# aj-prime/Elemental

Measured on AMD Instinct MI355X. Metric: distributed Gemm TFLOP/s (fp64/fp32) at 1/2/4/8 GPUs; % of MFMA peak, higher is better.
Workload: dtype f64; 1 GPU; C2: El::Gemm NN f64 m=n=k=32768, Grid 1x1; m=32768, n=32768, k=32768, grid=1x1, algorithm=SUMMA_C, blocksize=128, compute_panel=auto, parallelism=grid1x1, comm_reserved_cus=0

## Files before the change

### elemental_amd/_lib.py

```python
from __future__ import annotations

import ctypes
import os
from ctypes import (CFUNCTYPE, POINTER, c_char_p, c_double, c_float, c_int, c_int64, c_size_t,
                    c_ubyte, c_uint16, c_uint64, c_void_p)

_HERE = os.path.dirname(os.path.abspath(__file__))
LIB_PATH = os.path.join(_HERE, "libelemental_amd.so")

OK, ERR_LOGIC, ERR_HIP, ERR_COMM, ERR_RUNTIME, ERR_UNSUPPORTED, ERR_NO_DEVICE, ERR_SINGULAR = range(8)
ERR_NOT_HPD = 8
NORMAL, TRANSPOSE, ADJOINT = 0, 1, 2
MC, MD, MR, VC, VR, STAR, CIRC = range(7)
(GEMM_DEFAULT, GEMM_SUMMA_A_MS, GEMM_SUMMA_A, GEMM_SUMMA_B_MS, GEMM_SUMMA_B, GEMM_SUMMA_C_MS,
 GEMM_SUMMA_C, GEMM_SUMMA_DOT, GEMM_CANNON) = range(9)
ROW_MAJOR, COLUMN_MAJOR = 0, 1
LOWER, UPPER = 0, 1
LEFT, RIGHT = 0, 1
NON_UNIT, UNIT = 0, 1
CPU, GPU = 0, 1
F32, F64, F16, BF16 = 0, 1, 2, 3
I32, I64, U8 = 4, 5, 6
OP_SUM, OP_PROD, OP_MAX, OP_MIN = 0, 1, 2, 3
(MAP_IDENTITY, MAP_NEGATE, MAP_ABS, MAP_SQUARE, MAP_SQRT, MAP_EXP, MAP_LOG, MAP_RELU, MAP_SIGMOID,
 MAP_RECIP, MAP_TANH) = range(11)
(COMBINE_ADD, COMBINE_SUB, COMBINE_MUL, COMBINE_DIV, COMBINE_MAX, COMBINE_MIN, COMBINE_RELU_GRAD) = range(7)
FILE_AUTO, FILE_BINARY, FILE_BINARY_FLAT = 0, 3, 4
COLL_ALLGATHER, COLL_REDUCE_SCATTER, COLL_ALLTOALL, COLL_SENDRECV, COLL_BCAST, COLL_ALLREDUCE, \
    COLL_BARRIER = range(7)

HOST_COLL_FN = CFUNCTYPE(c_int, c_void_p, c_int, c_int, c_int, c_void_p, c_void_p, c_int64, c_int, c_int)
HOST_SPLIT_FN = CFUNCTYPE(c_int, c_void_p, c_int, c_int, c_int, POINTER(c_int), POINTER(c_int), POINTER(c_int))

_vp, _i, _i64, _d = c_void_p, c_int, c_int64, c_double
_SIGS = {
    "elx_last_error": (c_char_p, []),
    "elx_last_nonhpd_column": (_i, []),
    "elx_version": (_i, []),
    "elx_device_count": (_i, [POINTER(c_int)]),
    "elx_set_device": (_i, [_i]),
    "elx_get_device": (_i, [POINTER(c_int)]),
    "elx_device_synchronize": (_i, []),
    "elx_default_stream": (_i, [POINTER(c_void_p)]),
    "elx_comm_stream": (_i, [POINTER(c_void_p)]),
    "elx_reserved_cus": (_i, [POINTER(c_int)]),
    "elx_stream_create": (_i, [POINTER(c_void_p)]),
    "elx_stream_destroy": (_i, [_vp]),
    "elx_stream_synchronize": (_i, [_vp]),
    "elx_default_event": (_i, [POINTER(c_void_p)]),
    "elx_event_create": (_i, [POINTER(c_void_p)]),
    "elx_event_destroy": (_i, [_vp]),
    "elx_event_record": (_i, [_vp, _vp]),
    "elx_stream_wait_event": (_i, [_vp, _vp]),
    "elx_event_synchronize": (_i, [_vp]),
    "elx_pool_alloc": (_i, [POINTER(c_void_p), c_size_t, _vp]),
    "elx_pool_free": (_i, [_vp, _vp]),
    "elx_pool_trim": (_i, [c_size_t]),
    "elx_pool_stats": (_i, [POINTER(c_size_t), POINTER(c_size_t)]),
    "elx_pool_set_max_cached": (_i, [c_size_t]),
    "elx_pool_max_cached": (_i, [POINTER(c_size_t)]),
    "elx_pool_bin_bytes": (c_size_t, [c_size_t]),
    "elx_pool_bin_cacheable": (_i, [c_size_t]),
    "elx_pool_backing_reserved": (_i, [POINTER(c_size_t)]),
    "elx_memcpy_h2d": (_i, [_vp, _vp, c_size_t, _vp]),
    "elx_memcpy_d2h": (_i, [_vp, _vp, c_size_t, _vp]),
    "elx_memcpy_d2d": (_i, [_vp, _vp, c_size_t, _vp]),
    "elx_gemm_f64": (_i, [_i, _i, _i64, _i64, _i64, _d, _vp, _i64, _vp, _i64, _d, _vp, _i64, _vp]),
    "elx_gemm_f32": (_i, [_i, _i, _i64, _i64, _i64, c_float, _vp, _i64, _vp, _i64, c_float, _vp, _i64, _vp]),
# ... 218 lines not shown
```

### elemental_amd/csrc/capi.cpp

```cpp
#include "common.hpp"
#include "runtime/runtime.hpp"
#include "comm/comm.hpp"
#include "core/distmatrix.hpp"
#include "core/redist.hpp"
#include "core/gemm.hpp"
#include "core/lu.hpp"
#include "core/qr.hpp"
#include "core/random.hpp"
#include "core/io.hpp"
#include "core/exec.hpp"
#include <functional>
#include <string>

struct elx_comm_s { std::shared_ptr<elx::Comm> c; };
struct elx_grid_s { std::shared_ptr<elx::Grid> g; };
struct elx_dm_s { std::shared_ptr<elx::DistMatrix> m; };
struct elx_perm_s { elx::Permutation p; };

namespace elx {
namespace {
thread_local std::string g_last_error;

Dist ToDist(int d) {
    if (d < ELX_MC || d > ELX_CIRC) throw LogicError(Cat("invalid dist ", d));
// ... 29 lines not shown
using namespace elx;

extern "C" {

const char* elx_last_error(void) { return g_last_error.c_str(); }
int elx_last_nonhpd_column(void) { return g_last_nonhpd_column; }
int elx_version(void) { return 10000; }

int elx_device_count(int* count) {
    return Guard([&] {
        int n = 0;
        if (hipGetDeviceCount(&n) != hipSuccess) n = 0;
        *count = n;
    });
}
int elx_set_device(int device) { return Guard([&] { Runtime::Get().SetDevice(device); Runtime::Get().EnsureGPU(); }); }
int elx_get_device(int* device) { return Guard([&] { Runtime::Get().EnsureGPU(); *device = Runtime::Get().DeviceId(); }); }
int elx_device_synchronize(void) {
    return Guard([&] { Runtime::Get().EnsureGPU(); ELX_CHECK_HIP(hipDeviceSynchronize()); });
}
int elx_default_stream(void** stream) { return Guard([&] { *stream = Runtime::Get().ComputeStream(); }); }
int elx_comm_stream(void** stream) { return Guard([&] { *stream = Runtime::Get().CommStream(); }); }
int elx_reserved_cus(int* cus) { return Guard([&] { *cus = Runtime::Get().ReservedCUs(); }); }
int elx_stream_create(void** stream) {
    return Guard([&] {
        Runtime::Get().EnsureGPU();
        hipStream_t s;
        ELX_CHECK_HIP(hipStreamCreateWithFlags(&s, hipStreamNonBlocking));
        *stream = s;
    });
}
int elx_stream_destroy(void* stream) { return Guard([&] { ELX_CHECK_HIP(hipStreamDestroy(static_cast<hipStream_t>(stream))); }); }
int elx_stream_synchronize(void* stream) { return Guard([&] { ELX_CHECK_HIP(hipStreamSynchronize(S(stream))); }); }
int elx_default_event(void** event) {
    return Guard([&] {
        Runtime::Get().EnsureGPU();
        static hipEvent_t ev = [] {
            hipEvent_t e;
            ELX_CHECK_HIP(hipEventCreateWithFlags(&e, hipEventDisableTiming));
            return e;
        }();
        *event = ev;
    });
}
int elx_event_create(void** event) {
    return Guard([&] {
// ... 900 lines not shown
```

### elemental_amd/csrc/core/gemm.cpp

```cpp
#include "level3_internal.hpp"
#include <cstdlib>
#include "exec.hpp"
#include <algorithm>
#include <functional>
#include "../runtime/trace.hpp"
#include <vector>

namespace elx {

using namespace detail;

namespace {
std::vector<Int>& BlocksizeStack() {
    static std::vector<Int> s{128};
    return s;
}
Int g_compute_panel = 0;
int g_last_alg = ELX_GEMM_DEFAULT;
constexpr Int kDotBlock = 2000;
constexpr Int kDotBlockGPU = 2048;
Int DotBlockGPU() {
    static const Int v = [] { const char* e = getenv("ELX_DOT_BLOCK"); return e ? (Int)atoll(e) : kDotBlockGPU; }();
    return v;
}
// ... 125 lines not shown
        }
    }
};

int TeamCount(const DistMatrix& C, Int panels) {
    const int pool = StreamPoolSize();
    if (C.Dev() != Device::GPU || pool <= 1) return 1;
    return static_cast<int>(std::max<Int>(1, std::min<Int>(pool, panels)));
}

Int EffectivePanel(const Grid& g, Int K, DType t) {
    const Int nb = std::max<Int>(1, Blocksize());
    Int kc = g_compute_panel;
    const bool h16 = t == DType::F16 || t == DType::BF16;
    if (kc <= 0)
        kc = (g.Size() == 1) ? K : std::min<Int>(8192, std::max<Int>(2048, h16 ? K / 4 : K / 8));
    kc = std::max<Int>(nb, (kc + nb - 1) / nb * nb);
    return std::max<Int>(1, kc);
}

}

namespace detail {
void FenceStreams(hipStream_t from, hipStream_t to) {
    if (!from || !to || from == to) return;
    hipEvent_t ev;
    ELX_CHECK_HIP(hipEventCreateWithFlags(&ev, hipEventDisableTiming));
    ELX_CHECK_HIP(hipEventRecord(ev, from));
    ELX_CHECK_HIP(hipStreamWaitEvent(to, ev, 0));
    ELX_CHECK_HIP(hipEventDestroy(ev));
}

std::shared_ptr<const DistMatrix> ReadProxy(const DistMatrix& A, const DistMatrix& tgt, Dist cd, Dist rd,
                                            int calign, int ralign) {
    const bool ok = A.Dev() == tgt.Dev() && A.ColDist() == cd && A.RowDist() == rd &&
                    (calign < 0 || A.ColAlign() == calign) && (ralign < 0 || A.RowAlign() == ralign);
    if (ok) {
        if (A.Dev() != Device::GPU || A.Stream() == tgt.Stream())
            return std::shared_ptr<const DistMatrix>(&A, [](const DistMatrix*) {});
        auto V = DistMatrix::View(A, 0, A.Height(), 0, A.Width());
        V->SetStream(tgt.Stream());
        return V;
    }
    auto T = A.LikeOn(cd, rd, tgt.Dev());
    T->SetStream(tgt.Stream());
    const int ca = calign >= 0 ? calign : 0, ra = ralign >= 0 ? ralign : 0;
// ... 193 lines not shown
        const Int m = C.LocalHeight(), n = C.LocalWidth();
        const Int k = IsN(oA) ? a.LocalWidth() : a.LocalHeight();
        const double b_p = p == 0 ? beta : 1.0;
        if (m > 0 && n > 0 && k > 0) {
            const bool prof = gpu && Prof().on;
            Profiler::Rec rec{};
            if (prof) rec = Prof().Begin(cs);
            if (uplo >= 0)
                TrrkLocal(uplo == ELX_LOWER, !IsN(oA), !IsN(oB), k, alpha, a.Buffer(), a.LDim(), b.Buffer(), b.LDim(),
                          C, cs, trrk_tmp);
            else
                exec::Gemm(dev, C.Type(), !IsN(oA), !IsN(oB), m, n, k, alpha, a.Buffer(), a.LDim(), b.Buffer(),
                           b.LDim(), b_p, C.Buffer(), C.LDim(), cs);
            if (prof) Prof().End(rec, cs, 2.0 * m * n * k, Prof().gemm, call_id);
        } else if (p == 0) {
            Scale(beta, C);
        }
        if (gpu) {
            ELX_CHECK_HIP(hipEventRecord(s.done, cs));
            s.pending = true;
        }
    };
    if (np == 0) Scale(beta, C);
    if (np > 0) issue(0);
    for (int p = 0; p < np; ++p) {
        if (p + 1 < np) issue(p + 1);
        compute(p);
    }
    if (gpu) {
        FenceStreams(cs, ms);
        for (auto& s : slot) {
            s.ua.reset();
            s.ub.reset();
            s.va.reset();
            s.vb.reset();
            s.a.reset();
            s.b.reset();
            ELX_CHECK_HIP(hipEventDestroy(s.ready));
            ELX_CHECK_HIP(hipEventDestroy(s.done));
        }
    }
    Cp.Finish();
}
}

namespace {
// ... 12 lines not shown
    TeamViews tv(*Ap, *Bp, C0, TeamCount(C0, np));
    const int S = static_cast<int>(tv.v.size());
    const Dist a_cd = IsN(oA) ? Dist::MC : Dist::STAR, a_rd = IsN(oA) ? Dist::STAR : Dist::MC;
    const Dist b_cd = IsN(oB) ? Dist::STAR : Dist::MR, b_rd = IsN(oB) ? Dist::MR : Dist::STAR;
    struct TeamData { std::shared_ptr<DistMatrix> c, a, b; };
    std::vector<TeamData> td(S);
    for (int t = 0; t < S; ++t) {
        const DistMatrix& Ct = *tv.v[t].C;
        if (t == 0) {
            td[t].c = tv.v[t].C;
        } else {
            td[t].c = Ct.Like(Dist::MC, Dist::MR);
            td[t].c->Align(Ct.ColAlign(), Ct.RowAlign(), true);
            td[t].c->Resize(Ct.Height(), Ct.Width());
            Zero(*td[t].c);
        }
        td[t].a = tv.v[t].A->Like(a_cd, a_rd);
        td[t].b = tv.v[t].B->Like(b_cd, b_rd);
        if (IsN(oA)) td[t].a->AlignCols(Ct.ColAlign(), true); else td[t].a->AlignRows(Ct.ColAlign(), true);
        if (IsN(oB)) td[t].b->AlignRows(Ct.RowAlign(), true); else td[t].b->AlignCols(Ct.RowAlign(), true);
    }
    const Device dev = C0.Dev();
    const int call_id = Prof().calls++;
    for (Int p = 0; p < np; ++p) {
        const int t = static_cast<int>(p % S);
        const auto& v = tv.v[t];
        const DistMatrix& A = *v.A;
        const DistMatrix& B = *v.B;
        DistMatrix& Ct = *td[t].c;
        const Int k0 = p * kc, k1 = std::min(K, k0 + kc);
        auto Av = IsN(oA) ? DistMatrix::View(A, 0, A.Height(), k0, k1) : DistMatrix::View(A, k0, k1, 0, A.Width());
        auto Bv = IsN(oB) ? DistMatrix::View(B, k0, k1, 0, B.Width()) : DistMatrix::View(B, 0, B.Height(), k0, k1);
        std::shared_ptr<const DistMatrix> ua = Av, ub = Bv;
        if (!SameLocalLayout(*Av, a_cd, a_rd, td[t].a->ColAlign(), td[t].a->RowAlign())) {
            Copy(*Av, *td[t].a);
            ua = td[t].a;
        }
        if (!SameLocalLayout(*Bv, b_cd, b_rd, td[t].b->ColAlign(), td[t].b->RowAlign())) {
            Copy(*Bv, *td[t].b);
            ub = td[t].b;
        }
        const Int m = Ct.LocalHeight(), n = Ct.LocalWidth();
        const Int k = IsN(oA) ? ua->LocalWidth() : ua->LocalHeight();
        if (m > 0 && n > 0 && k > 0) {
            const bool prof = dev == Device::GPU && Prof().on;
            Profiler::Rec rec{};
// ... 355 lines not shown
```

### elemental_amd/csrc/kernels/gemm_f64g.hip

```cpp
#include <hip/hip_runtime.h>
#include <cstdint>
#include <cstdlib>
#include <type_traits>
#include "kernels.hpp"
#include "lds_dma.hpp"

namespace elx {
namespace kern {

namespace {

typedef double f64x4 __attribute__((ext_vector_type(4)));

constexpr int BK = 16, GROUP_M = 8;
constexpr bool RING64_DEFAULT = true;
template <int BM_, int WTM_ = 32, int SK_ = BK, int BN_ = 128, int WTN_ = 64>
struct Shape {
    static constexpr int BM = BM_, WTM = WTM_, MI = WTM_ / 16, WM = BM_ / WTM_, SK = SK_;
    static constexpr int BN = BN_, WTN = WTN_, NI = WTN_ / 16, WN = BN_ / WTN_, NW = WM * WN, NT = 64 * NW;
    static constexpr int IMGA = BM * SK * 8, IMGB = BN * SK * 8, STAGE = IMGA + IMGB;
    static constexpr int WAVES_PER_EU = BM_ == 64 && BN_ == 64 ? 4 : NW * (BM_ <= 128 && SK_ == 16 ? 2 : 1) / 4;
};

template <int SK>
__device__ __forceinline__ int swz_kc(int r) { return SK == 16 ? (r >> 1) & 7 : r & 15; }

struct GParams {
    i64 m, n, k;
    double alpha, beta;
    const double* A; i64 lda;
    const double* B; i64 ldb;
    double* C; i64 ldc;
    int tiles_m, tiles_n;
    i64 kchunk, zstride;
    int group_m;
    int xcd_remap;
};

__device__ __forceinline__ void tile_of(int bid, int nwg, int tiles_m, int tiles_n, int group_m, int remap, int& tm,
                                        int& tn) {
    const int xcd = bid & 7, q = nwg >> 3, r = nwg & 7;
    const int wg = remap ? (xcd < r ? xcd * (q + 1) : r * (q + 1) + (xcd - r) * q) + (bid >> 3) : bid;
    const int per_group = group_m * tiles_n;
    const int group = wg / per_group;
    const int first_m = group * group_m;
    const int gsz = min(tiles_m - first_m, group_m);
    const int inner = wg - group * per_group;
    tm = first_m + inner % gsz;
    tn = inner / gsz;
}

template <bool BUF, bool KC, int ROWS, int NW, int SK>
__device__ __forceinline__ void stage_img(const double* X, i64 ld, i64 rows, i64 R, i64 k0, lds_char* img, int w,
                                          int l) {
    constexpr int NINS = ROWS * SK * 8 / 1024;
    constexpr int CPR = SK / 2, RPI = 64 / CPR;
    const DmaSrc<BUF, double> src(KC ? X + R * ld + k0 : X + R + k0 * ld, (KC ? ROWS : SK) * ld * 8);
#pragma unroll
    for (int q = 0; q < NINS / NW; ++q) {
// ... 221 lines not shown
        if constexpr (NP > 0) {
            if (i >= H + OFF && (i - H - OFF) % SP == 0 && (i - H - OFF) / SP < NP) {
                const int u = u0 + (i - H - OFF) / SP;
                if constexpr (SB) piece<BT, UN, BUF, KCB>(p.B, p.ldb, n0, k0, pc.offB[u], pc.gB[u], w + 4 * u, st);
                else piece<BT, UN, BUF, KCA>(p.A, p.lda, m0, k0, pc.offA[u], pc.gA[u], w + 4 * u, st);
            }
        }
        __builtin_amdgcn_sched_barrier(0);
    }
}
}

template <int BT, int UN, bool KCA, bool KCB, bool BETA0, bool BUF>
__global__ __launch_bounds__(256, (ring::RG<BT, UN>::MINB)) void gemm_f64r_kernel(GParams p) {
    using namespace ring;
    using G = RG<BT, UN>;
    constexpr int RBK = G::RBK, UNIT = G::UNIT, WT = G::WT, MI = G::MI, NKS = G::NKS, NPW = G::NPW;
    constexpr int NPA = NPW / (NKS / 2);
    __shared__ __attribute__((aligned(1024))) char lds_raw[NSLOT * UNIT];
    lds_char* lds = (lds_char*)lds_raw;
    const int tid = threadIdx.x, l = tid & 63;
    const int w = __builtin_amdgcn_readfirstlane(tid >> 6);
    const int wr = w >> 1, wc = w & 1;
    int tm, tn;
    tile_of(blockIdx.x, gridDim.x, p.tiles_m, p.tiles_n, p.group_m, p.xcd_remap, tm, tn);
    const i64 m0 = (i64)tm * BT, n0 = (i64)tn * BT;
    {
        const i64 kz0 = (i64)blockIdx.y * p.kchunk;
        p.k = min(p.kchunk, p.k - kz0);
        p.A += KCA ? kz0 : kz0 * p.lda;
        p.B += KCB ? kz0 : kz0 * p.ldb;
        p.C += (i64)blockIdx.y * p.zstride;
    }
    Pieces<BT, UN> pc;
#pragma unroll
    for (int u = 0; u < NPW; ++u) {
        pc.gA[u] = piece_off<BT, UN, KCA>(w + 4 * u, l, m0, p.m, p.lda);
        pc.gB[u] = piece_off<BT, UN, KCB>(w + 4 * u, l, n0, p.n, p.ldb);
        pc.offA[u] = (int)(pc.gA[u] * 8);
        pc.offB[u] = (int)(pc.gB[u] * 8);
    }
    f64x4 acc[MI][MI];
#pragma unroll
    for (int a = 0; a < MI; ++a)
#pragma unroll
        for (int b = 0; b < MI; ++b) acc[a][b] = f64x4{0, 0, 0, 0};

    const int nt = (int)(p.k / RBK);
    auto kt = [&](int t) { return (i64)min(t, nt - 1) * RBK; };
#pragma unroll
    for (int t = 0; t < 2; ++t) {
#pragma unroll
        for (int u = 0; u < NPW; ++u)
            piece<BT, UN, BUF, KCA>(p.A, p.lda, m0, kt(t), pc.offA[u], pc.gA[u], w + 4 * u, lds + 2 * t * UNIT);
#pragma unroll
        for (int u = 0; u < NPW; ++u)
            piece<BT, UN, BUF, KCB>(p.B, p.ldb, n0, kt(t), pc.offB[u], pc.gB[u], w + 4 * u, lds + (2 * t + 1) * UNIT);
    }
    wait_cnt<2 * NPW, NOWAIT_LGKM>();
    dma_barrier();
    Ops<BT, UN> X, Y;
#pragma unroll
    for (int q = 0; q < MI; ++q) {
        X.a[q] = ropnd<BT, UN, KCA>(lds, wr * WT + q * 16, 0, l);
        X.b[q] = ropnd<BT, UN, KCB>(lds + UNIT, wc * WT + q * 16, 0, l);
    }
    wait_cnt<NOWAIT_VM, 0>();
    auto ktile = [&](auto jc, int t) {
        constexpr int J = decltype(jc)::value;
        constexpr int sA = 2 * J % NSLOT, sB = (2 * J + 1) % NSLOT, sA1 = (2 * J + 2) % NSLOT,
                      sB1 = (2 * J + 3) % NSLOT, st0 = (2 * J + 4) % NSLOT, st1 = (2 * J + 5) % NSLOT;
        lds_char* rA = lds + sA * UNIT;
        lds_char* rB = lds + sB * UNIT;
        const i64 k2 = kt(t + 2);
        auto ks = [&](auto sc) {
            constexpr int S = decltype(sc)::value;
            constexpr int NP = S < NKS / 2 ? NPA : 0;
            if constexpr (S % 2 == 0)
                ring::kstep<BT, UN, KCA, KCB, BUF, false, NP>(p, m0, n0, w, l, wr, wc, pc, rA, rB, S + 1,
                                                          lds + st0 * UNIT, S * NPA, k2, acc, X, Y);
            else
                ring::kstep<BT, UN, KCA, KCB, BUF, false, NP>(p, m0, n0, w, l, wr, wc, pc, rA, rB, S + 1,
                                                          lds + st0 * UNIT, S * NPA, k2, acc, Y, X);
            if constexpr (S < NKS - 2) wait_cnt<NOWAIT_VM, 0>();
        };
        ks(std::integral_constant<int, 0>{});
        ks(std::integral_constant<int, 1>{});
        ks(std::integral_constant<int, 2>{});
        if constexpr (NKS == 8) {
            ks(std::integral_constant<int, 3>{});
            ks(std::integral_constant<int, 4>{});
            ks(std::integral_constant<int, 5>{});
            ks(std::integral_constant<int, 6>{});
        }
        wait_cnt<NPW, 0>();
        dma_barrier();
        ring::kstep<BT, UN, KCA, KCB, BUF, true, NPW>(p, m0, n0, w, l, wr, wc, pc, lds + sA1 * UNIT, lds + sB1 * UNIT,
                                                  0, lds + st1 * UNIT, 0, k2, acc, Y, X);
        wait_cnt<NOWAIT_VM, 0>();
    };
    for (int t = 0; t < nt; t += NSLOT) {
        ktile(std::integral_constant<int, 0>{}, t);
        if (t + 1 < nt) ktile(std::integral_constant<int, 1>{}, t + 1);
        if (t + 2 < nt) ktile(std::integral_constant<int, 2>{}, t + 2);
        if (t + 3 < nt) ktile(std::integral_constant<int, 3>{}, t + 3);
        if (t + 4 < nt) ktile(std::integral_constant<int, 4>{}, t + 4);
    }
    asm volatile("s_waitcnt vmcnt(0)" ::: "memory");

    const int g = l >> 4, c = l & 15;
    const i64 ib = m0 + wr * WT + c, jb = n0 + wc * WT + g;
    if (m0 + BT <= p.m && n0 + BT <= p.n) {
#pragma unroll
        for (int mi = 0; mi < MI; ++mi) {
            double cv[MI][4];
            if (!BETA0) {
#pragma unroll
                for (int ni = 0; ni < MI; ++ni)
#pragma unroll
                    for (int r = 0; r < 4; ++r) cv[ni][r] = p.C[(jb + ni * 16 + 4 * r) * p.ldc + ib + mi * 16];
            }
#pragma unroll
            for (int ni = 0; ni < MI; ++ni)
#pragma unroll
                for (int r = 0; r < 4; ++r) {
                    const double v = p.alpha * acc[mi][ni][r];
                    p.C[(jb + ni * 16 + 4 * r) * p.ldc + ib + mi * 16] = BETA0 ? v : v + p.beta * cv[ni][r];
                }
        }
        return;
    }
#pragma unroll
    for (int mi = 0; mi < MI; ++mi)
#pragma unroll
        for (int ni = 0; ni < MI; ++ni) {
            const i64 i = ib + mi * 16;
            if (i >= p.m) continue;
#pragma unroll
            for (int r = 0; r < 4; ++r) {
                const i64 j = jb + ni * 16 + 4 * r;
                if (j < p.n) {
                    const double v = p.alpha * acc[mi][ni][r];
                    double* cp = p.C + j * p.ldc + i;
                    *cp = BETA0 ? v : v + p.beta * *cp;
                }
            }
        }
}

template <typename K>
hipError_t launch(K kernel, dim3 grid, int nt, const GParams& p, hipStream_t s) {
    hipLaunchKernelGGL(kernel, grid, dim3(nt), 0, s, p);
    return hipGetLastError();
}


template <typename SH, bool KCA, bool KCB, bool BUF>
hipError_t launch_b(const GParams& p, dim3 grid, hipStream_t s) {
    if (p.beta == 0.0) return launch(gemm_f64g_kernel<SH, KCA, KCB, true, BUF>, grid, SH::NT, p, s);
    return launch(gemm_f64g_kernel<SH, KCA, KCB, false, BUF>, grid, SH::NT, p, s);
}

template <typename SH, bool KCA, bool KCB>
hipError_t launch_g(GParams p, hipStream_t s) {
    p.tiles_m = (int)((p.m + SH::BM - 1) / SH::BM);
    p.tiles_n = (int)((p.n + SH::BN - 1) / SH::BN);
    const dim3 grid(p.tiles_m * p.tiles_n, (unsigned)((p.k + p.kchunk - 1) / p.kchunk));
    static const bool global_only = [] { const char* v = getenv("ELX_F64G_STAGE"); return v && v[0] == 'g'; }();
    if (!global_only && dma_fits(KCA ? SH::BM : SH::SK, p.lda, 8) && dma_fits(KCB ? SH::BN : SH::SK, p.ldb, 8))
        return launch_b<SH, KCA, KCB, true>(p, grid, s);
    return launch_b<SH, KCA, KCB, false>(p, grid, s);
}

template <int BT, int UN, bool KCA, bool KCB>
hipError_t launch_r(GParams p, hipStream_t s) {
    constexpr int RBK = ring::RG<BT, UN>::RBK;
    p.tiles_m = (int)((p.m + BT - 1) / BT);
    p.tiles_n = (int)((p.n + BT - 1) / BT);
    const dim3 grid(p.tiles_m * p.tiles_n, (unsigned)((p.k + p.kchunk - 1) / p.kchunk));
    const char* stg = getenv("ELX_F64G_STAGE");
    const bool buf = !(stg && stg[0] == 'g') && dma_fits(KCA ? BT : RBK, p.lda, 8) &&
                     dma_fits(KCB ? BT : RBK, p.ldb, 8);
    if (p.beta == 0.0) {
        if (buf) return launch(gemm_f64r_kernel<BT, UN, KCA, KCB, true, true>, grid, 256, p, s);
        return launch(gemm_f64r_kernel<BT, UN, KCA, KCB, true, false>, grid, 256, p, s);
    }
    if (buf) return launch(gemm_f64r_kernel<BT, UN, KCA, KCB, false, true>, grid, 256, p, s);
    return launch(gemm_f64r_kernel<BT, UN, KCA, KCB, false, false>, grid, 256, p, s);
}

template <typename SH>
hipError_t launch_shape(bool kca, bool kcb, const GParams& p, hipStream_t s) {
    if (kca) return kcb ? launch_g<SH, true, true>(p, s) : launch_g<SH, true, false>(p, s);
    return kcb ? launch_g<SH, false, true>(p, s) : launch_g<SH, false, false>(p, s);
}

bool al16(const void* q) { return (reinterpret_cast<uintptr_t>(q) & 15) == 0; }

bool t64_tiles(i64 m, i64 n, i64 k) {
    static const int v = [] { const char* e = getenv("ELX_F64G_T64"); return e ? atoi(e) : 1; }();
    if (v == 1 && (m + 127) / 128 * ((n + 127) / 128) == 256 && k / 32 * 32 <= 4096) return true;
    return prefer_t64(v, m, n, 255);
}

int ring_bt(i64 m, i64 n, i64 k) {
    const char* e = getenv("ELX_F64G_RING");
    const int v = e ? atoi(e) : RING64_DEFAULT ? 3 : 1;
    if (t64_tiles(m, n, k)) return (v & 2) ? 64 : 0;
    return (v & 1) ? 128 : 0;
}

}

DmaPlan gemm_f64_lds_dma_plan(bool ta, bool tb, i64 m, i64 n, i64 k, const double* A, i64 lda, const double* B,
                              i64 ldb) {
    const bool kca = ta, kcb = !tb;
    const bool ok = k >= BK && al16(A) && al16(B) && lda % 2 == 0 && ldb % 2 == 0 && (kca || (m % 2 == 0 && m >= 2)) &&
                    (kcb || (n % 2 == 0 && n >= 2)) && m < (1ll << 31) && n < (1ll << 31);
    const int bt = ring_bt(m, n, k);
    if (bt == 128) return dma_plan(ok && k >= 32, (m + 127) / 128 * ((n + 127) / 128), k, 32, 256);
    if (t64_tiles(m, n, k)) return dma_plan(ok, (m + 63) / 64 * ((n + 63) / 64), k, BK, bt == 64 ? 1024 : 512);
    return dma_plan(ok, (m + 127) / 128 * ((n + 127) / 128), k, BK);
}

hipError_t gemm_f64_lds_dma(bool ta, bool tb, i64 m, i64 n, i64 kmain, i64 kchunk, double alpha, const double* A,
                            i64 lda, const double* B, i64 ldb, double beta, double* C, i64 ldc, hipStream_t s) {
    static const int gm = [] {
        const char* v = getenv("ELX_F64G_GROUP");
        const int g = v ? atoi(v) : GROUP_M;
        return g >= 1 ? g : 1;
    }();
    static const int rm = [] { const char* v = getenv("ELX_F64G_REMAP"); return v ? atoi(v) : 1; }();
    GParams p{m, n, kmain, alpha, beta, A, lda, B, ldb, C, ldc, 0, 0, kchunk, m * n, gm, rm};
    static const int t64w = [] { const char* v = getenv("ELX_F64G_T64W"); return v ? atoi(v) : 0; }();
    const int bt = ring_bt(m, n, kmain);
    if (bt == 128 && kmain % 32 == 0 && kchunk % 32 == 0) {
        if (ta) return !tb ? launch_r<128, 32768, true, true>(p, s) : launch_r<128, 32768, true, false>(p, s);
        return !tb ? launch_r<128, 32768, false, true>(p, s) : launch_r<128, 32768, false, false>(p, s);
    }
    if (bt == 64 && kmain % 16 == 0 && kchunk % 16 == 0) {
        if (ta) return !tb ? launch_r<64, 8192, true, true>(p, s) : launch_r<64, 8192, true, false>(p, s);
        return !tb ? launch_r<64, 8192, false, true>(p, s) : launch_r<64, 8192, false, false>(p, s);
    }
    if (t64_tiles(m, n, kmain)) {
        if (t64w == 8 || (t64w != 4 && !ta)) return launch_shape<Shape<64, 32, BK, 64, 16>>(ta, !tb, p, s);
        return launch_shape<Shape<64, 32, BK, 64, 32>>(ta, !tb, p, s);
    }
    static const int wtm_env = [] { const char* v = getenv("ELX_F64G_WTM"); return v ? atoi(v) : 0; }();
    const i64 grid_wgs = (m + 127) / 128 * ((n + 127) / 128) * ((kmain + kchunk - 1) / kchunk);
    const int wtm = wtm_env ? wtm_env : ((!ta && tb) || grid_wgs <= 256) ? 32 : 64;
    if (wtm == 64) return launch_shape<Shape<128, 64>>(ta, !tb, p, s);
    return launch_shape<Shape<128>>(ta, !tb, p, s);
}

}
}
// ... 1 lines not shown
```

### elemental_amd/csrc/kernels/kernels.hpp

```cpp
#pragma once
#include <hip/hip_runtime.h>
#include <algorithm>
#include <cstdint>
#include <cstdlib>

namespace elx {
namespace kern {

hipError_t workspace_alloc(void** p, size_t bytes, hipStream_t s);
hipError_t workspace_free(void* p, hipStream_t s);

using i64 = int64_t;

template <typename T>
hipError_t gemm_mfma(bool ta, bool tb, i64 m, i64 n, i64 k, T alpha, const T* A, i64 lda,
                     const T* B, i64 ldb, T beta, T* C, i64 ldc, hipStream_t s);
struct DmaPlan {
    bool use;
    i64 kmain, kchunk;
    int nz;
};
inline DmaPlan dma_plan(bool ok, i64 tiles, i64 k, int bk, i64 slots = 512) {
    DmaPlan d{false, 0, 0, 1};
    if (!ok) return d;
    d.kmain = k / bk * bk;
    if (tiles >= slots) {
        d.use = true;
        d.kchunk = d.kmain;
        return d;
    }
    static const i64 min_env = [] { const char* v = getenv("ELX_DMA_MIN_CHUNK"); return v ? atoll(v) : 0ll; }();
    const i64 min_chunk = min_env >= bk ? min_env : tiles < 256 ? 256 : 2048;
    i64 z = (2 * slots + tiles - 1) / tiles;
    if (tiles > 32 && tiles < 256) z = tiles <= 200 ? 4 : 2;
    z = z < d.kmain / min_chunk ? z : d.kmain / min_chunk;
    z = z < 16 ? z : 16;
    if (z < 2) {
        static const bool few = [] { const char* v = getenv("ELX_DMA_FEW"); return !v || v[0] != '0'; }();
        d.use = few && d.kmain > 0;
        d.kchunk = d.kmain;
        return d;
    }
    d.use = true;
    d.kchunk = ((d.kmain + z - 1) / z + bk - 1) / bk * bk;
    d.nz = (int)((d.kmain + d.kchunk - 1) / d.kchunk);
    return d;
}
inline bool prefer_t64(int mode, i64 m, i64 n, i64 small = 255) {
    if (mode == 0 || mode == 2) return mode == 2;
    const i64 t128 = (m + 127) / 128 * ((n + 127) / 128), t64 = (m + 63) / 64 * ((n + 63) / 64);
    if (t128 <= small) return true;
    const auto bal = [](i64 t) { return (double)t / (double)(256 * ((t + 255) / 256)); };
    return 0.95 * bal(t64) > bal(t128);
}
DmaPlan gemm_f64_lds_dma_plan(bool ta, bool tb, i64 m, i64 n, i64 k, const double* A, i64 lda, const double* B,
                              i64 ldb);
hipError_t gemm_f64_lds_dma(bool ta, bool tb, i64 m, i64 n, i64 kmain, i64 kchunk, double alpha, const double* A,
                            i64 lda, const double* B, i64 ldb, double beta, double* C, i64 ldc, hipStream_t s);
DmaPlan gemm_f32_lds_dma_plan(bool ta, bool tb, i64 m, i64 n, i64 k, const float* A, i64 lda, const float* B,
                              i64 ldb);
hipError_t gemm_f32_lds_dma(bool ta, bool tb, i64 m, i64 n, i64 kmain, i64 kchunk, float alpha, const float* A,
                            i64 lda, const float* B, i64 ldb, float beta, float* C, i64 ldc, hipStream_t s);
struct H16Plan { int wm; i64 nz, kchunk; };
inline H16Plan h16_plan(i64 m, i64 n, i64 kmain, bool tn = false) {
    constexpr i64 BK = 64;
    const char* tv = getenv("ELX_H16_TILE");
    const int force = tv ? atoi(tv) : 0;
    auto tiles_of = [&](i64 bm) { return ((m + bm - 1) / bm) * ((n + bm - 1) / bm); };
    auto util = [](i64 t, i64 slots) { return (double)t / (double)(((t + slots - 1) / slots) * slots); };
    H16Plan pl;
    if (force == 64 || force == 128 || force == 160 || force == 192 || force == 224 || force == 256) {
        pl.wm = force / 32;
    } else if (tiles_of(256) < 128) {
        pl.wm = tn && tiles_of(160) >= 224 ? 5 : 4;
        const i64 t4 = tiles_of(128);
        if (pl.wm == 4 && t4 >= 64 && t4 < 256) {
            const i64 z4 = t4 <= 64 && kmain >= 8 * BK ? std::min<i64>((256 + t4 - 1) / t4, kmain / (16 * BK)) : 1;
// ... 119 lines not shown
```

### elemental_amd/csrc/runtime/runtime.cpp

```cpp
#include "runtime.hpp"
#include "../kernels/kernels.hpp"
#include <algorithm>
#include <cstdio>
#include <cstdlib>
#include <limits>
#include <vector>

namespace elx {

Runtime& Runtime::Get() {
    static Runtime* rt = new Runtime();
    return *rt;
}

void Runtime::SetDevice(int dev) {
    std::lock_guard<std::mutex> lk(mu_);
    if (gpu_ready_ && dev != device_)
        throw LogicError(Cat("elx: device already initialised as ", device_, "; cannot switch to ", dev));
    device_ = dev;
}

void Runtime::EnsureGPU() {
    if (gpu_ready_) return;
    std::lock_guard<std::mutex> lk(mu_);
// ... 10 lines not shown
        device_ = local % n;
    }
    ELX_CHECK_HIP(hipSetDevice(device_));
    hipDeviceProp_t prop;
    ELX_CHECK_HIP(hipGetDeviceProperties(&prop, device_));
    if (std::string(prop.gcnArchName).rfind("gfx950", 0) != 0)
        throw NoDeviceError(Cat("elx: device ", device_, " is ", prop.gcnArchName,
                                "; this build targets gfx950 (MI355X) only"));
    const int ncu = prop.multiProcessorCount;
    if (const char* e = std::getenv("ELX_COMM_CUS")) reserved_cus_ = std::max(0, std::atoi(e));
    if (reserved_cus_ > 0 && reserved_cus_ < ncu) {
        std::vector<uint32_t> mask((ncu + 31) / 32, 0);
        for (int i = 0; i < ncu; ++i) mask[i / 32] |= 1u << (i % 32);
        const int slice = ncu / reserved_cus_;
        for (int r = 0; r < reserved_cus_; ++r) {
            const int i = std::min(ncu - 1, r * slice + (r % 8) % std::max(1, slice));
            mask[i / 32] &= ~(1u << (i % 32));
        }
        ELX_CHECK_HIP(hipExtStreamCreateWithCUMask(&compute_, static_cast<uint32_t>(mask.size()), mask.data()));
    } else {
        reserved_cus_ = 0;
        ELX_CHECK_HIP(hipStreamCreateWithFlags(&compute_, hipStreamNonBlocking));
    }
    int lo = 0, hi = 0;
    ELX_CHECK_HIP(hipDeviceGetStreamPriorityRange(&lo, &hi));
    const char* pe = getenv("ELX_COMM_PRIORITY");
    ELX_CHECK_HIP(hipStreamCreateWithPriority(&comm_, hipStreamNonBlocking, pe && atoi(pe) == 0 ? lo : hi));
    if (!max_cached_set_) {
        for (const char* v : {"ELX_POOL_MAX_CACHED", "H_CUB_MAX_CACHED_SIZE"}) {
            if (const char* e = std::getenv(v)) { max_cached_ = std::strtoull(e, nullptr, 10); break; }
        }
    }
    gpu_ready_ = true;
}

namespace {
struct BinConfig {
    bool cub = false;
    unsigned growth = 2, min_bin = 1, max_bin = ~0u;
    bool debug = false;
};
unsigned EnvUint(const char* name, unsigned def, bool& set) {
    const char* e = std::getenv(name);
    if (!e || !*e) return def;
    set = true;
    return static_cast<unsigned>(std::strtoul(e, nullptr, 10));
// ... 333 lines not shown
```

### include/elemental_amd.h

```cpp
#ifndef ELEMENTAL_AMD_H
#define ELEMENTAL_AMD_H

#include <stddef.h>
#include <stdint.h>

#ifdef __cplusplus
extern "C" {
#endif

#define ELX_OK                  0
#define ELX_ERR_LOGIC           1
#define ELX_ERR_HIP             2
#define ELX_ERR_COMM            3
#define ELX_ERR_RUNTIME         4
#define ELX_ERR_UNSUPPORTED     5
#define ELX_ERR_NO_DEVICE       6
#define ELX_ERR_SINGULAR        7
#define ELX_ERR_NOT_HPD         8

#define ELX_NORMAL     0
#define ELX_TRANSPOSE  1
#define ELX_ADJOINT    2
#define ELX_MC    0
#define ELX_MD    1
// ... 37 lines not shown
#define ELX_MAP_LOG      6
#define ELX_MAP_RELU     7
#define ELX_MAP_SIGMOID  8
#define ELX_MAP_RECIP    9
#define ELX_MAP_TANH     10
#define ELX_COMBINE_ADD       0
#define ELX_COMBINE_SUB       1
#define ELX_COMBINE_MUL       2
#define ELX_COMBINE_DIV       3
#define ELX_COMBINE_MAX       4
#define ELX_COMBINE_MIN       5
#define ELX_COMBINE_RELU_GRAD 6

const char* elx_last_error(void);
int elx_last_nonhpd_column(void);
int elx_version(void);
int elx_device_count(int* count);
int elx_set_device(int device);
int elx_get_device(int* device);
int elx_device_synchronize(void);
int elx_default_stream(void** stream);
int elx_comm_stream(void** stream);
int elx_reserved_cus(int* cus);
int elx_stream_create(void** stream);
int elx_stream_destroy(void* stream);
int elx_stream_synchronize(void* stream);
int elx_default_event(void** event);
int elx_event_create(void** event);
int elx_event_destroy(void* event);
int elx_event_record(void* event, void* stream);
int elx_stream_wait_event(void* stream, void* event);
int elx_event_synchronize(void* event);

int elx_pool_alloc(void** ptr, size_t bytes, void* stream);
int elx_pool_free(void* ptr, void* stream);
int elx_pool_trim(size_t bytes_to_keep);
int elx_pool_stats(size_t* bytes_reserved, size_t* bytes_in_use);
int elx_pool_set_max_cached(size_t bytes);
int elx_pool_max_cached(size_t* bytes);
size_t elx_pool_bin_bytes(size_t bytes);
int elx_pool_bin_cacheable(size_t bytes);
int elx_pool_backing_reserved(size_t* bytes);
int elx_memcpy_h2d(void* dst, const void* src, size_t bytes, void* stream);
int elx_memcpy_d2h(void* dst, const void* src, size_t bytes, void* stream);
int elx_memcpy_d2d(void* dst, const void* src, size_t bytes, void* stream);

// ... 257 lines not shown
```

Baseline: 76.53 TFLOP/s.

## Add persistent tile walk to f64 GEMM kernel for multi-GPU pipelined runs

```diff
diff --git a/elemental_amd/_lib.py b/elemental_amd/_lib.py
--- a/elemental_amd/_lib.py
+++ b/elemental_amd/_lib.py
@@ -44,6 +44,9 @@
     "elx_default_stream": (_i, [POINTER(c_void_p)]),
     "elx_comm_stream": (_i, [POINTER(c_void_p)]),
     "elx_reserved_cus": (_i, [POINTER(c_int)]),
+    "elx_f64_tile_walk_cap": (_i, [POINTER(c_int)]),
+    "elx_set_f64_tile_walk_cap": (_i, [_i]),
+    "elx_f64_tile_walk_last": (_i, [POINTER(c_int), POINTER(c_int), POINTER(c_int)]),
     "elx_stream_create": (_i, [POINTER(c_void_p)]),
     "elx_stream_destroy": (_i, [_vp]),
     "elx_stream_synchronize": (_i, [_vp]),
diff --git a/elemental_amd/csrc/capi.cpp b/elemental_amd/csrc/capi.cpp
--- a/elemental_amd/csrc/capi.cpp
+++ b/elemental_amd/csrc/capi.cpp
@@ -75,6 +75,11 @@
 int elx_default_stream(void** stream) { return Guard([&] { *stream = Runtime::Get().ComputeStream(); }); }
 int elx_comm_stream(void** stream) { return Guard([&] { *stream = Runtime::Get().CommStream(); }); }
 int elx_reserved_cus(int* cus) { return Guard([&] { *cus = Runtime::Get().ReservedCUs(); }); }
+int elx_f64_tile_walk_cap(int* cap) { return Guard([&] { *cap = kern::f64_tile_walk_cap(); }); }
+int elx_set_f64_tile_walk_cap(int cap) { return Guard([&] { kern::set_f64_tile_walk_cap(cap); }); }
+int elx_f64_tile_walk_last(int* slots, int* cap, int* grid) {
+    return Guard([&] { kern::f64_tile_walk_last(slots, cap, grid); });
+}
 int elx_stream_create(void** stream) {
     return Guard([&] {
         Runtime::Get().EnsureGPU();
diff --git a/elemental_amd/csrc/core/gemm.cpp b/elemental_amd/csrc/core/gemm.cpp
--- a/elemental_amd/csrc/core/gemm.cpp
+++ b/elemental_amd/csrc/core/gemm.cpp
@@ -171,6 +171,19 @@
 }
 
 namespace detail {
+constexpr int kWalkCapPipelined = 4;
+struct WalkCapGuard {
+    int saved = -1;
+    WalkCapGuard(const Grid& g, Device dev) {
+        if (dev != Device::GPU || g.Size() <= 1 || Runtime::Get().ReservedCUs() > 0) return;
+        saved = kern::f64_tile_walk_cap();
+        kern::set_f64_tile_walk_cap(saved > 0 ? std::min(saved, kWalkCapPipelined) : kWalkCapPipelined);
+    }
+    ~WalkCapGuard() { if (saved >= 0) kern::set_f64_tile_walk_cap(saved); }
+    WalkCapGuard(const WalkCapGuard&) = delete;
+    WalkCapGuard& operator=(const WalkCapGuard&) = delete;
+};
+
 void FenceStreams(hipStream_t from, hipStream_t to) {
     if (!from || !to || from == to) return;
     hipEvent_t ev;
@@ -410,6 +423,7 @@
         }
     };
     if (np == 0) Scale(beta, C);
+    const WalkCapGuard walk_cap(g, dev);
     if (np > 0) issue(0);
     for (int p = 0; p < np; ++p) {
         if (p + 1 < np) issue(p + 1);
@@ -468,6 +482,7 @@
     }
     const Device dev = C0.Dev();
     const int call_id = Prof().calls++;
+    const WalkCapGuard walk_cap(C0.G(), dev);
     for (Int p = 0; p < np; ++p) {
         const int t = static_cast<int>(p % S);
         const auto& v = tv.v[t];
diff --git a/elemental_amd/csrc/kernels/gemm_f64g.hip b/elemental_amd/csrc/kernels/gemm_f64g.hip
--- a/elemental_amd/csrc/kernels/gemm_f64g.hip
+++ b/elemental_amd/csrc/kernels/gemm_f64g.hip
@@ -1,4 +1,6 @@
 #include <hip/hip_runtime.h>
+#include <algorithm>
+#include <atomic>
 #include <cstdint>
 #include <cstdlib>
 #include <type_traits>
@@ -35,6 +37,7 @@
     i64 kchunk, zstride;
     int group_m;
     int xcd_remap;
+    int walk_s, walk_t;
 };
 
 __device__ __forceinline__ void tile_of(int bid, int nwg, int tiles_m, int tiles_n, int group_m, int remap, int& tm,
@@ -302,9 +305,6 @@
     const int tid = threadIdx.x, l = tid & 63;
     const int w = __builtin_amdgcn_readfirstlane(tid >> 6);
     const int wr = w >> 1, wc = w & 1;
-    int tm, tn;
-    tile_of(blockIdx.x, gridDim.x, p.tiles_m, p.tiles_n, p.group_m, p.xcd_remap, tm, tn);
-    const i64 m0 = (i64)tm * BT, n0 = (i64)tn * BT;
     {
         const i64 kz0 = (i64)blockIdx.y * p.kchunk;
         p.k = min(p.kchunk, p.k - kz0);
@@ -312,40 +312,47 @@
         p.B += KCB ? kz0 : kz0 * p.ldb;
         p.C += (i64)blockIdx.y * p.zstride;
     }
-    Pieces<BT, UN> pc;
-#pragma unroll
-    for (int u = 0; u < NPW; ++u) {
-        pc.gA[u] = piece_off<BT, UN, KCA>(w + 4 * u, l, m0, p.m, p.lda);
-        pc.gB[u] = piece_off<BT, UN, KCB>(w + 4 * u, l, n0, p.n, p.ldb);
-        pc.offA[u] = (int)(pc.gA[u] * 8);
-        pc.offB[u] = (int)(pc.gB[u] * 8);
-    }
-    f64x4 acc[MI][MI];
-#pragma unroll
-    for (int a = 0; a < MI; ++a)
-#pragma unroll
-        for (int b = 0; b < MI; ++b) acc[a][b] = f64x4{0, 0, 0, 0};
-
     const int nt = (int)(p.k / RBK);
     auto kt = [&](int t) { return (i64)min(t, nt - 1) * RBK; };
-#pragma unroll
-    for (int t = 0; t < 2; ++t) {
-#pragma unroll
-        for (int u = 0; u < NPW; ++u)
-            piece<BT, UN, BUF, KCA>(p.A, p.lda, m0, kt(t), pc.offA[u], pc.gA[u], w + 4 * u, lds + 2 * t * UNIT);
-#pragma unroll
-        for (int u = 0; u < NPW; ++u)
-            piece<BT, UN, BUF, KCB>(p.B, p.ldb, n0, kt(t), pc.offB[u], pc.gB[u], w + 4 * u, lds + (2 * t + 1) * UNIT);
-    }
+    const int tiles = p.tiles_m * p.tiles_n;
+    i64 m0, n0;
+    Pieces<BT, UN> pc;
+    auto stage_tile = [&](int v) {
+        int tm, tn;
+        tile_of(v, tiles, p.tiles_m, p.tiles_n, p.group_m, p.xcd_remap, tm, tn);
+        m0 = (i64)tm * BT;
+        n0 = (i64)tn * BT;
+#pragma unroll
+        for (int u = 0; u < NPW; ++u) {
+            pc.gA[u] = piece_off<BT, UN, KCA>(w + 4 * u, l, m0, p.m, p.lda);
+            pc.gB[u] = piece_off<BT, UN, KCB>(w + 4 * u, l, n0, p.n, p.ldb);
+            pc.offA[u] = (int)(pc.gA[u] * 8);
+            pc.offB[u] = (int)(pc.gB[u] * 8);
+        }
+#pragma unroll
+        for (int t = 0; t < 2; ++t) {
+#pragma unroll
+            for (int u = 0; u < NPW; ++u)
+                piece<BT, UN, BUF, KCA>(p.A, p.lda, m0, kt(t), pc.offA[u], pc.gA[u], w + 4 * u, lds + 2 * t * UNIT);
+#pragma unroll
+            for (int u = 0; u < NPW; ++u)
+                piece<BT, UN, BUF, KCB>(p.B, p.ldb, n0, kt(t), pc.offB[u], pc.gB[u], w + 4 * u,
+                                        lds + (2 * t + 1) * UNIT);
+        }
+    };
+    f64x4 acc[MI][MI];
+    auto zero_acc = [&] {
+#pragma unroll
+        for (int a = 0; a < MI; ++a)
+#pragma unroll
+            for (int b = 0; b < MI; ++b) acc[a][b] = f64x4{0, 0, 0, 0};
+    };
+    Ops<BT, UN> X, Y;
+    const unsigned wg = blockIdx.x, walk_s = p.walk_s, walk_t = p.walk_t;
+    stage_tile(walk_t == 1 ? (int)wg : (int)tile_walk_index<unsigned>(wg, 0, walk_s, walk_t));
+    zero_acc();
     wait_cnt<2 * NPW, NOWAIT_LGKM>();
     dma_barrier();
-    Ops<BT, UN> X, Y;
-#pragma unroll
-    for (int q = 0; q < MI; ++q) {
-        X.a[q] = ropnd<BT, UN, KCA>(lds, wr * WT + q * 16, 0, l);
-        X.b[q] = ropnd<BT, UN, KCB>(lds + UNIT, wc * WT + q * 16, 0, l);
-    }
-    wait_cnt<NOWAIT_VM, 0>();
     auto ktile = [&](auto jc, int t) {
         constexpr int J = decltype(jc)::value;
         constexpr int sA = 2 * J % NSLOT, sB = (2 * J + 1) % NSLOT, sA1 = (2 * J + 2) % NSLOT,
@@ -379,53 +386,77 @@
                                                   0, lds + st1 * UNIT, 0, k2, acc, Y, X);
         wait_cnt<NOWAIT_VM, 0>();
     };
-    for (int t = 0; t < nt; t += NSLOT) {
-        ktile(std::integral_constant<int, 0>{}, t);
-        if (t + 1 < nt) ktile(std::integral_constant<int, 1>{}, t + 1);
-        if (t + 2 < nt) ktile(std::integral_constant<int, 2>{}, t + 2);
-        if (t + 3 < nt) ktile(std::integral_constant<int, 3>{}, t + 3);
-        if (t + 4 < nt) ktile(std::integral_constant<int, 4>{}, t + 4);
-    }
-    asm volatile("s_waitcnt vmcnt(0)" ::: "memory");
-
-    const int g = l >> 4, c = l & 15;
-    const i64 ib = m0 + wr * WT + c, jb = n0 + wc * WT + g;
-    if (m0 + BT <= p.m && n0 + BT <= p.n) {
-#pragma unroll
-        for (int mi = 0; mi < MI; ++mi) {
-            double cv[MI][4];
-            if (!BETA0) {
+    for (unsigned step = 1;; ++step) {
+#pragma unroll
+        for (int q = 0; q < MI; ++q) {
+            X.a[q] = ropnd<BT, UN, KCA>(lds, wr * WT + q * 16, 0, l);
+            X.b[q] = ropnd<BT, UN, KCB>(lds + UNIT, wc * WT + q * 16, 0, l);
+        }
+        wait_cnt<NOWAIT_VM, 0>();
+        for (int t = 0; t < nt; t += NSLOT) {
+            ktile(std::integral_constant<int, 0>{}, t);
+            if (t + 1 < nt) ktile(std::integral_constant<int, 1>{}, t + 1);
+            if (t + 2 < nt) ktile(std::integral_constant<int, 2>{}, t + 2);
+            if (t + 3 < nt) ktile(std::integral_constant<int, 3>{}, t + 3);
+            if (t + 4 < nt) ktile(std::integral_constant<int, 4>{}, t + 4);
+        }
+        asm volatile("s_waitcnt vmcnt(0)" ::: "memory");
+
+        const i64 em0 = m0, en0 = n0;
+        bool more = false;
+        if constexpr (BT == 128) {
+            const unsigned vn = step < walk_t ? tile_walk_index<unsigned>(wg, step, walk_s, walk_t) : tiles;
+            more = vn < (unsigned)tiles;
+            if (more) {
+                wait_cnt<NOWAIT_VM, 0>();
+                dma_barrier();
+                stage_tile((int)vn);
+            }
+        }
+
+        const int g = l >> 4, c = l & 15;
+        const i64 ib = em0 + wr * WT + c, jb = en0 + wc * WT + g;
+        if (em0 + BT <= p.m && en0 + BT <= p.n) {
+#pragma unroll
+            for (int mi = 0; mi < MI; ++mi) {
+                double cv[MI][4];
+                if (!BETA0) {
+#pragma unroll
+                    for (int ni = 0; ni < MI; ++ni)
+#pragma unroll
+                        for (int r = 0; r < 4; ++r) cv[ni][r] = p.C[(jb + ni * 16 + 4 * r) * p.ldc + ib + mi * 16];
+                }
 #pragma unroll
                 for (int ni = 0; ni < MI; ++ni)
 #pragma unroll
-                    for (int r = 0; r < 4; ++r) cv[ni][r] = p.C[(jb + ni * 16 + 4 * r) * p.ldc + ib + mi * 16];
+                    for (int r = 0; r < 4; ++r) {
+                        const double v = p.alpha * acc[mi][ni][r];
+                        p.C[(jb + ni * 16 + 4 * r) * p.ldc + ib + mi * 16] = BETA0 ? v : v + p.beta * cv[ni][r];
+                    }
             }
-#pragma unroll
-            for (int ni = 0; ni < MI; ++ni)
-#pragma unroll
-                for (int r = 0; r < 4; ++r) {
-                    const double v = p.alpha * acc[mi][ni][r];
-                    p.C[(jb + ni * 16 + 4 * r) * p.ldc + ib + mi * 16] = BETA0 ? v : v + p.beta * cv[ni][r];
+        } else {
+#pragma unroll
+            for (int mi = 0; mi < MI; ++mi)
+#pragma unroll
+                for (int ni = 0; ni < MI; ++ni) {
+                    const i64 i = ib + mi * 16;
+                    if (i >= p.m) continue;
+#pragma unroll
+                    for (int r = 0; r < 4; ++r) {
+                        const i64 j = jb + ni * 16 + 4 * r;
+                        if (j < p.n) {
+                            const double v = p.alpha * acc[mi][ni][r];
+                            double* cp = p.C + j * p.ldc + i;
+                            *cp = BETA0 ? v : v + p.beta * *cp;
+                        }
+                    }
                 }
         }
-        return;
-    }
-#pragma unroll
-    for (int mi = 0; mi < MI; ++mi)
-#pragma unroll
-        for (int ni = 0; ni < MI; ++ni) {
-            const i64 i = ib + mi * 16;
-            if (i >= p.m) continue;
-#pragma unroll
-            for (int r = 0; r < 4; ++r) {
-                const i64 j = jb + ni * 16 + 4 * r;
-                if (j < p.n) {
-                    const double v = p.alpha * acc[mi][ni][r];
-                    double* cp = p.C + j * p.ldc + i;
-                    *cp = BETA0 ? v : v + p.beta * *cp;
-                }
-            }
-        }
+        if (!more) break;
+        zero_acc();
+        asm volatile("s_waitcnt vmcnt(0)" ::: "memory");
+        dma_barrier();
+    }
 }
 
 template <typename K>
@@ -452,12 +483,40 @@
     return launch_b<SH, KCA, KCB, false>(p, grid, s);
 }
 
+std::atomic<int> g_walk_cap{1}, g_walk_reserved{0};
+std::atomic<int> g_walk_last[3];
+
+TileWalk walk_of(i64 tiles, int nz) {
+    static const int ncu = [] {
+        int dev = 0, n = 0;
+        if (hipGetDevice(&dev) != hipSuccess ||
+            hipDeviceGetAttribute(&n, hipDeviceAttributeMultiprocessorCount, dev) != hipSuccess || n < 8)
+            n = 256;
+        return n;
+    }();
+    const char* se = getenv("ELX_F64G_SLOTS");
+    const char* pe = getenv("ELX_F64G_PERSIST");
+    const int slots = se ? atoi(se) : ncu - g_walk_reserved.load(std::memory_order_relaxed);
+    const int cap = pe ? std::max(1, atoi(pe)) : g_walk_cap.load(std::memory_order_relaxed);
+    return tile_walk_plan(tiles, nz, slots, cap);
+}
+
 template <int BT, int UN, bool KCA, bool KCB>
 hipError_t launch_r(GParams p, hipStream_t s) {
     constexpr int RBK = ring::RG<BT, UN>::RBK;
     p.tiles_m = (int)((p.m + BT - 1) / BT);
     p.tiles_n = (int)((p.n + BT - 1) / BT);
-    const dim3 grid(p.tiles_m * p.tiles_n, (unsigned)((p.k + p.kchunk - 1) / p.kchunk));
+    const i64 tiles = (i64)p.tiles_m * p.tiles_n;
+    const unsigned nz = (unsigned)((p.k + p.kchunk - 1) / p.kchunk);
+    const TileWalk wk = BT == 128 ? walk_of(tiles, (int)nz) : TileWalk{8, 1};
+    p.walk_s = wk.S;
+    p.walk_t = wk.T;
+    const dim3 grid((unsigned)tile_walk_grid(tiles, wk.S, wk.T), nz);
+    if (BT == 128) {
+        g_walk_last[0] = wk.S;
+        g_walk_last[1] = wk.T;
+        g_walk_last[2] = (int)grid.x;
+    }
     const char* stg = getenv("ELX_F64G_STAGE");
     const bool buf = !(stg && stg[0] == 'g') && dma_fits(KCA ? BT : RBK, p.lda, 8) &&
                      dma_fits(KCB ? BT : RBK, p.ldb, 8);
@@ -478,7 +537,8 @@
 bool al16(const void* q) { return (reinterpret_cast<uintptr_t>(q) & 15) == 0; }
 
 bool t64_tiles(i64 m, i64 n, i64 k) {
-    static const int v = [] { const char* e = getenv("ELX_F64G_T64"); return e ? atoi(e) : 1; }();
+    const char* e = getenv("ELX_F64G_T64");
+    const int v = e ? atoi(e) : 1;
     if (v == 1 && (m + 127) / 128 * ((n + 127) / 128) == 256 && k / 32 * 32 <= 4096) return true;
     return prefer_t64(v, m, n, 255);
 }
@@ -490,6 +550,15 @@
     return (v & 1) ? 128 : 0;
 }
 
+}
+
+void set_f64_tile_walk_cap(int cap) { g_walk_cap = std::max(0, cap); }
+int f64_tile_walk_cap() { return g_walk_cap; }
+void set_f64_tile_walk_reserved_cus(int cus) { g_walk_reserved = std::max(0, cus); }
+void f64_tile_walk_last(int* S, int* T, int* grid) {
+    *S = g_walk_last[0];
+    *T = g_walk_last[1];
+    *grid = g_walk_last[2];
 }
 
 DmaPlan gemm_f64_lds_dma_plan(bool ta, bool tb, i64 m, i64 n, i64 k, const double* A, i64 lda, const double* B,
@@ -511,7 +580,7 @@
         return g >= 1 ? g : 1;
     }();
     static const int rm = [] { const char* v = getenv("ELX_F64G_REMAP"); return v ? atoi(v) : 1; }();
-    GParams p{m, n, kmain, alpha, beta, A, lda, B, ldb, C, ldc, 0, 0, kchunk, m * n, gm, rm};
+    GParams p{m, n, kmain, alpha, beta, A, lda, B, ldb, C, ldc, 0, 0, kchunk, m * n, gm, rm, 8, 1};
     static const int t64w = [] { const char* v = getenv("ELX_F64G_T64W"); return v ? atoi(v) : 0; }();
     const int bt = ring_bt(m, n, kmain);
     if (bt == 128 && kmain % 32 == 0 && kchunk % 32 == 0) {
diff --git a/elemental_amd/csrc/kernels/kernels.hpp b/elemental_amd/csrc/kernels/kernels.hpp
--- a/elemental_amd/csrc/kernels/kernels.hpp
+++ b/elemental_amd/csrc/kernels/kernels.hpp
@@ -29,7 +29,8 @@
         d.kchunk = d.kmain;
         return d;
     }
-    static const i64 min_env = [] { const char* v = getenv("ELX_DMA_MIN_CHUNK"); return v ? atoll(v) : 0ll; }();
+    const char* min_v = getenv("ELX_DMA_MIN_CHUNK");
+    const i64 min_env = min_v ? atoll(min_v) : 0ll;
     const i64 min_chunk = min_env >= bk ? min_env : tiles < 256 ? 256 : 2048;
     i64 z = (2 * slots + tiles - 1) / tiles;
     if (tiles > 32 && tiles < 256) z = tiles <= 200 ? 4 : 2;
@@ -53,6 +54,23 @@
     const auto bal = [](i64 t) { return (double)t / (double)(256 * ((t + 255) / 256)); };
     return 0.95 * bal(t64) > bal(t128);
 }
+template <typename I = i64>
+constexpr I tile_walk_index(I b, I i, I S, I T) { return (b / S) * S * T + i * S + b % S; }
+constexpr i64 tile_walk_grid(i64 tiles, i64 S, i64 T) {
+    return tiles / (S * T) * S + (tiles % (S * T) < S ? tiles % (S * T) : S);
+}
+constexpr i64 tile_walk_rounds(i64 tiles, i64 S) { return (tiles + S - 1) / S; }
+struct TileWalk { int S, T; };
+constexpr TileWalk tile_walk_plan(i64 tiles, int nz, int slots, int cap) {
+    const int S = slots / 8 * 8 < 8 ? 8 : slots / 8 * 8;
+    if (nz > 1 || tiles <= S || cap == 1) return TileWalk{S, 1};
+    const i64 r = tile_walk_rounds(tiles, S);
+    return TileWalk{S, (int)(cap > 0 && cap < r ? cap : r)};
+}
+void set_f64_tile_walk_cap(int cap);
+int f64_tile_walk_cap();
+void set_f64_tile_walk_reserved_cus(int cus);
+void f64_tile_walk_last(int* S, int* T, int* grid);
 DmaPlan gemm_f64_lds_dma_plan(bool ta, bool tb, i64 m, i64 n, i64 k, const double* A, i64 lda, const double* B,
                               i64 ldb);
 hipError_t gemm_f64_lds_dma(bool ta, bool tb, i64 m, i64 n, i64 kmain, i64 kchunk, double alpha, const double* A,
diff --git a/elemental_amd/csrc/runtime/runtime.cpp b/elemental_amd/csrc/runtime/runtime.cpp
--- a/elemental_amd/csrc/runtime/runtime.cpp
+++ b/elemental_amd/csrc/runtime/runtime.cpp
@@ -56,6 +56,7 @@
         reserved_cus_ = 0;
         ELX_CHECK_HIP(hipStreamCreateWithFlags(&compute_, hipStreamNonBlocking));
     }
+    kern::set_f64_tile_walk_reserved_cus(reserved_cus_);
     int lo = 0, hi = 0;
     ELX_CHECK_HIP(hipDeviceGetStreamPriorityRange(&lo, &hi));
     const char* pe = getenv("ELX_COMM_PRIORITY");
diff --git a/include/elemental_amd.h b/include/elemental_amd.h
--- a/include/elemental_amd.h
+++ b/include/elemental_amd.h
@@ -83,6 +83,9 @@
 int elx_default_stream(void** stream);
 int elx_comm_stream(void** stream);
 int elx_reserved_cus(int* cus);
+int elx_f64_tile_walk_cap(int* cap);
+int elx_set_f64_tile_walk_cap(int cap);
+int elx_f64_tile_walk_last(int* slots, int* cap, int* grid);
 int elx_stream_create(void** stream);
 int elx_stream_destroy(void* stream);
 int elx_stream_synchronize(void* stream);
```

Result: no change. 76.96 TFLOP/s, median of 6 (+0.6%).
